# JonathanLehner/korali

Hardware: AMD Instinct MI355X
Metric: CMA-ES generations/sec + samples/sec, 128-dim Rosenbrock λ=4096, 1→8 GPUs (higher is better)
Workload: dtype f64; 1 GPU; C2: CMA-ES, 128-dim negative Rosenbrock, lambda=4096, mu=2048 Logarithmic, x0=0, sigma0=1, seed 1337; one experiment per GPU; population=4096, variables=128, covariance_update=exact, parallelism=replicas1

## Files before the change

### include/korali_amd.h

```cpp
#ifndef KORALI_AMD_H
#define KORALI_AMD_H

#include <stddef.h>
#include <stdint.h>

#ifdef __cplusplus
extern "C" {
#endif

#define KG_ABI_VERSION 8

const char *kg_last_error(void);
int kg_abi_version(void);
int kg_device_count(int *count);

typedef struct kg_cmaes_s *kg_cmaes_t;

enum kg_mu_type { KG_MU_LOGARITHMIC = 0, KG_MU_LINEAR = 1, KG_MU_EQUAL = 2, KG_MU_PROPORTIONAL = 3 };
enum kg_objective { KG_OBJ_NEGATIVE_ROSENBROCK = 0, KG_OBJ_NEGATIVE_ACKLEY = 1, KG_OBJ_NEGATIVE_SPHERE = 2 };
enum kg_cov_mode { KG_COV_EXACT = 0, KG_COV_MFMA = 1 };

typedef struct {
  size_t variable_count;
  size_t population_size;
// ... 11 lines not shown
  const double *initial_value;
  const double *initial_std;
  const double *min_std_update;
  uint64_t normal_seed;
  uint64_t uniform_seed;
  int cov_mode;
  int device;
  int store_bdz;
  int eigen_device_chase;
  int shard_rank;
  int shard_count;
  int use_gradients;
  double gradient_step_size;
  const double *granularity;
  size_t constraint_count;
  size_t viability_population_size;
  size_t viability_mu_value;
  double max_covariance_matrix_corrections;
  double target_success_rate;
  double covariance_matrix_adaption_strength;
  double global_success_learning_rate;
} kg_cmaes_cfg;

int kg_cmaes_create(const kg_cmaes_cfg *cfg, kg_cmaes_t *out);

typedef int (*kg_constraint_fn)(const double *X, size_t rows, size_t N, const size_t *ids, double *out, void *ctx);
int kg_cmaes_set_constraints(kg_cmaes_t h, kg_constraint_fn fn, void *ctx);
int kg_cmaes_prepare_constrained(kg_cmaes_t h, size_t generation);
int kg_cmaes_population_size(kg_cmaes_t h, size_t *lambda, size_t *mu);
int kg_cmaes_destroy(kg_cmaes_t h);
int kg_cmaes_initialize(kg_cmaes_t h);
int kg_cmaes_sample(kg_cmaes_t h);
int kg_cmaes_eval_builtin(kg_cmaes_t h, int objective);
int kg_cmaes_get_candidates(kg_cmaes_t h, double *X, size_t ld);
int kg_cmaes_set_fitness(kg_cmaes_t h, const double *F);
int kg_cmaes_set_log_posterior(kg_cmaes_t h, const double *F);
int kg_cmaes_set_gradients(kg_cmaes_t h, const double *G);
int kg_cmaes_update(kg_cmaes_t h, size_t generation);
int kg_cmaes_generation(kg_cmaes_t h, size_t generation, int objective);
int kg_cmaes_begin_sample(kg_cmaes_t h);
#define KG_TERMINATION_FIELDS 9
int kg_cmaes_wait_termination_fields(kg_cmaes_t h, double *out);
int kg_cmaes_update_partial(kg_cmaes_t h, size_t generation);
int kg_cmaes_shard_row_count(kg_cmaes_t h, size_t *count);
int kg_cmaes_update_rows(kg_cmaes_t h, size_t generation);
int kg_cmaes_update_finalize(kg_cmaes_t h, size_t generation);
int kg_cmaes_synchronize(kg_cmaes_t h);
int kg_cmaes_field_size(kg_cmaes_t h, const char *name, size_t *n);
int kg_cmaes_get_field(kg_cmaes_t h, const char *name, double *out, size_t n);
int kg_cmaes_set_field(kg_cmaes_t h, const char *name, const double *in, size_t n);
int kg_cmaes_get_fields(kg_cmaes_t h, const char *const *names, size_t count, double *out);
int kg_cmaes_get_sorting_index(kg_cmaes_t h, uint64_t *out);
int kg_cmaes_get_rng(kg_cmaes_t h, int which, void *state5000);
int kg_cmaes_set_rng(kg_cmaes_t h, int which, const void *state5000);
int kg_cmaes_device_ptr(kg_cmaes_t h, const char *name, void **ptr);
int kg_cmaes_stream(kg_cmaes_t h, void **stream);
int kg_cmaes_profile(kg_cmaes_t h, int enable);
int kg_cmaes_profile_read(kg_cmaes_t h, const char *stage, double *ms_total, size_t *count);
int kg_cmaes_profile_mark(kg_cmaes_t h, const char *stage, int phase);

typedef struct kg_dea_s *kg_dea_t;

enum kg_dea_mutation_rule { KG_DEA_MUTATION_FIXED = 0, KG_DEA_MUTATION_SELF_ADAPTIVE = 1 };
enum kg_dea_parent_rule { KG_DEA_PARENT_RANDOM = 0, KG_DEA_PARENT_BEST = 1 };
enum kg_dea_accept_rule {
  KG_DEA_ACCEPT_BEST = 0,
// ... 193 lines not shown
```

### korali_amd/csrc/kg_cmaes.hip

```cpp
#include <cmath>
#include <cstdio>
#include <cstdlib>
#include <cstring>
#include <map>
#include <string>
#include <tuple>
#include <vector>

#include "../../include/korali_amd.h"
#include "kg_common.hpp"
#include "kg_chains.hpp"
#include "kg_eigen.hpp"
#include "kg_rng.hpp"
#include <chrono>

namespace kg {


struct CmaesScalars {
  double sigma, trace, effectiveMu, cumulativeCovariance, sigmaCumulationFactor, dampFactor, chiSquareNumber;
  double psNorm, bestEverValue, previousBestEverValue, previousBestValue, currentBestValue;
  double currentMinStd, currentMaxStd, maxDiagC, minDiagC, minEig, maxEig;
  double infeasibleSampleCount, bestValidSample, modelEvaluationCount, hsig, eigenFailures;
  double ccov1, ccovmu;
// ... 99 lines not shown
      C[i * N + i] = v * v;
    }
    double mn = D[0], mx = D[0];
    for (int i = 1; i < N; i++) {
      if (D[i] < mn) mn = D[i];
      if (D[i] > mx) mx = D[i];
    }
    sc->minEig = mn * mn;
    sc->maxEig = mx * mx;
    double maxd = C[0], mind = C[0];
    for (int i = 1; i < N; ++i)
      if (maxd < C[i * N + i]) maxd = C[i * N + i];
    for (int i = 1; i < N; ++i)
      if (mind > C[i * N + i]) mind = C[i * N + i];
    sc->maxDiagC = maxd;
    sc->minDiagC = mind;
    if (full) {
      sc->infeasibleSampleCount = 0;
      sc->psNorm = 0.0;
      sc->currentMinStd = INFINITY;
      sc->currentMaxStd = -INFINITY;
      sc->hsigPowGen = -1.0;
    }
  }
}

constexpr int TR_BK = 32, TR_XCD = 8;
template <int BM, int BN>
inline unsigned tr_grid(int rows, int N) {
  const int nbm = (rows + BM - 1) / BM, nbn = (N + BN - 1) / BN;
  return (unsigned)(((nbm + TR_XCD - 1) / TR_XCD) * TR_XCD * nbn);
}
template <int BM, int BN>
__global__ void __launch_bounds__(256) k_transform(int N, int rows, int diagonal, const double *__restrict__ Z,
                                                   const double *__restrict__ B, const double *__restrict__ D,
                                                   const double *__restrict__ mean, CmaesScalars *__restrict__ sc,
                                                   const double *__restrict__ lb, const double *__restrict__ ub,
                                                   double *__restrict__ X, double *__restrict__ BDZ,
                                                   int *__restrict__ infeas, int no_reserve, int mirrored) {
  constexpr int PR = BM / 8, PC = BN / 32, ZL = BM * TR_BK / 256, BL = BN * TR_BK / 256;
  __shared__ __attribute__((aligned(16))) double Za[TR_BK][BM + 2];
  __shared__ __attribute__((aligned(16))) double Bt[TR_BK][BN + 2];
  const int tid = threadIdx.x;
  const int nbn = (N + BN - 1) / BN;
  const int xcd = blockIdx.x % TR_XCD, j = blockIdx.x / TR_XCD;
  const int rt = (j / nbn) * TR_XCD + xcd, ct = j % nbn;
  const int i0 = rt * BM, d0 = ct * BN;
  if (i0 >= rows) return;
  const int tx = tid & 31, ty = tid >> 5;
  const double sigma = sc->sigma;
  double acc[PR][PC];
#pragma unroll
  for (int p = 0; p < PR; p++)
#pragma unroll
    for (int q = 0; q < PC; q++) acc[p][q] = 0.0;
  if (!diagonal) {
    double zr[ZL], br[BL];
    auto load = [&](int k0) {
#pragma unroll
      for (int r = 0; r < ZL; r++) {
        const int q = tid + 256 * r, c = q / TR_BK, e = k0 + q % TR_BK, i = i0 + c;
        double z = 0.0;
        if (i < rows && e < N) {
          z = Z[(size_t)(mirrored ? (i >> 1) : i) * N + e];
          if (mirrored && (i & 1)) z = -z;
          z = D[e] * z;
        }
        zr[r] = z;
      }
#pragma unroll
      for (int r = 0; r < BL; r++) {
        const int q = tid + 256 * r, dd = q / TR_BK, e = k0 + q % TR_BK, d = d0 + dd;
        br[r] = (d < N && e < N) ? B[(size_t)d * N + e] : 0.0;
      }
    };
    auto store = [&]() {
#pragma unroll
      for (int r = 0; r < ZL; r++) {
        const int q = tid + 256 * r;
        Za[q % TR_BK][q / TR_BK] = zr[r];
      }
// ... 32 lines not shown
          for (int u = 0; u < 8; u++) t[u] = b[(g + u) % PC] * a[(g + u) / PC];
#pragma unroll
          for (int u = 0; u < 8; u++) acc[(g + u) / PC][(g + u) % PC] += t[u];
        }
      };
      fetch(a0, b0, 0);
      if (kmax == TR_BK) {
#pragma unroll 1
        for (int kk = 0; kk < TR_BK - 2; kk += 2) {
          fetch(a1, b1, kk + 1);
          madd(a0, b0);
          fetch(a0, b0, kk + 2);
          madd(a1, b1);
        }
        fetch(a1, b1, TR_BK - 1);
        madd(a0, b0);
        madd(a1, b1);
      } else {
#pragma unroll 1
        for (int kk = 0; kk < kmax; kk++) {
          fetch(a0, b0, kk);
          madd(a0, b0);
        }
      }
      __syncthreads();
      if (more) {
        store();
        __syncthreads();
      }
    }
  }
#pragma unroll
  for (int p = 0; p < PR; p++) {
    const int i = i0 + ty * PR + p;
    if (i >= rows) continue;
    int bad = 0;
#pragma unroll
    for (int q = 0; q < PC; q++) {
      const int d = d0 + tx * PC + q;
      if (d >= N) continue;
      double zd = 0.0;
      if (diagonal) {
        zd = Z[(size_t)(mirrored ? (i >> 1) : i) * N + d];
        if (mirrored && (i & 1)) zd = -zd;
      }
      const double bdz = diagonal ? D[d] * zd : acc[p][q];
      const double x = mean[d] + sigma * bdz;
      X[(size_t)i * N + d] = x;
      if (BDZ) BDZ[(size_t)i * N + d] = bdz;
      if (!isfinite(x) || x < lb[d] || x > ub[d]) bad = 1;
    }
    if (bad) {
      if (no_reserve)
        atomicOr(&sc->errors, KG_ERR_DRAW_GUARD);
      else
        atomicOr(&infeas[i], 1);
    }
  }
}

constexpr int PS_T = 64;
__global__ void __launch_bounds__(256) k_prescale_t(int N, int rows, int ldz, const double *__restrict__ Z,
                                                    const double *__restrict__ D, int mirrored,
                                                    double *__restrict__ dzT) {
  __shared__ double t[PS_T][PS_T + 1];
  const int i0 = blockIdx.x * PS_T, k0 = blockIdx.y * PS_T, tid = threadIdx.x;
#pragma unroll 4
  for (int r = 0; r < PS_T * PS_T / 256; r++) {
    const int q = tid + 256 * r, ii = q / PS_T, kk = q % PS_T, i = i0 + ii, k = k0 + kk;
    double z = 0.0;
    if (i < rows && k < N) {
      z = Z[(size_t)(mirrored ? (i >> 1) : i) * N + k];
      if (mirrored && (i & 1)) z = -z;
      z = D[k] * z;
    }
    t[ii][kk] = z;
  }
  __syncthreads();
#pragma unroll 4
  for (int r = 0; r < PS_T * PS_T / 256; r++) {
    const int q = tid + 256 * r, kk = q / PS_T, ii = q % PS_T, k = k0 + kk;
    if (k < N) dzT[(size_t)k * ldz + i0 + ii] = t[ii][kk];
  }
}
inline int sc_ldz(size_t rows) { return (int)((rows + 127) / 128 * 128); }
template <int C, int RPL>
inline unsigned trs_grid(int rows, int N) {
  const int nrt = (rows + 64 * RPL - 1) / (64 * RPL), ncg = (N + 4 * C - 1) / (4 * C);
  return (unsigned)(((nrt + TR_XCD - 1) / TR_XCD) * TR_XCD * ncg);
}
inline int transform_width(int N) {
// ... 188 lines not shown
        const int d = d0 + dd;
        if (obj == KG_OBJ_NEGATIVE_ROSENBROCK) {
          if (d > 0) {
            const double tt = x - prev * prev;
            const double u = 1 - prev;
            r0 += 100 * (tt * tt) + u * u;
          }
          prev = x;
        } else if (obj == KG_OBJ_NEGATIVE_ACKLEY) {
          r0 += x * x;
          r1 += ctile[tid][dd];
        } else {
          r0 += x * x;
        }
      }
    }
    __syncthreads();
  }
  if (tid >= OB_C || i >= lam) return;
  double f;
  if (obj == KG_OBJ_NEGATIVE_ROSENBROCK)
    f = -r0;
  else if (obj == KG_OBJ_NEGATIVE_ACKLEY) {
    const double s1 = r0 / (double)N, s2 = r1 / (double)N;
    const double e1 = 20. * exp_cr(-0.2 * sqrt(s1));
    const double e2 = exp_cr(s2);
    f = e1 + e2 - 20. - 2.718281828459045;
  } else
    f = -0.5 * r0;
  F[i] = f;
  if (!isfinite(f)) atomicOr(&sc->errors, KG_ERR_NONFINITE_F);
}

constexpr int OB2_R = 64, OB2_NC = 32;
__host__ __device__ inline size_t ob2_lds_bytes(int N) {
  return ((size_t)OB2_R * (N + 1) + 2 * 2 * (size_t)OB2_R * (OB2_NC + 1)) * sizeof(double);
}
__global__ void __launch_bounds__(256) k_objective2(int N, int lam, int obj, const double *__restrict__ X,
                                                    double *__restrict__ F, CmaesScalars *sc, double addEvals) {
  extern __shared__ __attribute__((aligned(16))) double ob2[];
  if (blockIdx.x == 0 && threadIdx.x == 0) sc->modelEvaluationCount += addEvals;
  const int tid = threadIdx.x, lane = tid & 63, wid = __builtin_amdgcn_readfirstlane(tid >> 6);
  const int ld = N + 1, c0 = blockIdx.x * OB2_R;
  double *Xs = ob2;
  double *Ta = Xs + (size_t)OB2_R * ld;
  double *Tb = Ta + 2 * (size_t)OB2_R * (OB2_NC + 1);
  const int tot = OB2_R * N;
  for (int q0 = tid; q0 < tot; q0 += 32 * 256) {
    double v[32];
#pragma unroll
    for (int u = 0; u < 32; u++) {
      const int q = q0 + u * 256, r = q / N, d = q - r * N;
      v[u] = (q < tot && c0 + r < lam) ? X[(size_t)(c0 + r) * N + d] : 0.0;
    }
#pragma unroll
    for (int u = 0; u < 32; u++) {
      const int q = q0 + u * 256, r = q / N, d = q - r * N;
      if (q < tot) Xs[(size_t)r * ld + d] = v[u];
    }
  }
  __syncthreads();
  const int nch = (N + OB2_NC - 1) / OB2_NC;
  const double cc = 2. * 3.141592653589793;
  auto form = [&](int ch) {
    const int b = ch & 1, d0 = ch * OB2_NC, dn = min(OB2_NC, N - d0);
    double *ta = Ta + (size_t)b * OB2_R * (OB2_NC + 1) + (size_t)lane * (OB2_NC + 1);
    double *tb = Tb + (size_t)b * OB2_R * (OB2_NC + 1) + (size_t)lane * (OB2_NC + 1);
    const double *xr = Xs + (size_t)lane * ld;
    if (obj != KG_OBJ_NEGATIVE_ACKLEY) {
      constexpr int PU = (OB2_NC + 2) / 3;
      double xs[PU], xp[PU];
#pragma unroll
      for (int u = 0; u < PU; u++) {
        const int dd = wid - 1 + 3 * u, d = d0 + dd;
        xs[u] = dd < dn ? xr[d] : 0.0;
        xp[u] = (dd < dn && d > 0) ? xr[d - 1] : 0.0;
      }
#pragma unroll
      for (int u = 0; u < PU; u++) {
        const int dd = wid - 1 + 3 * u, d = d0 + dd;
        if (dd >= dn) break;
        const double x = xs[u];
        if (obj == KG_OBJ_NEGATIVE_ROSENBROCK) {
          if (d > 0) {
            const double prev = xp[u];
            const double tt = x - prev * prev;
            const double uu = 1 - prev;
            ta[dd] = 100 * (tt * tt) + uu * uu;
          }
        } else {
          ta[dd] = x * x;
        }
      }
      return;
    }
    for (int dd = wid - 1; dd < dn; dd += 3) {
      const int d = d0 + dd;
      const double x = xr[d];
      if (obj == KG_OBJ_NEGATIVE_ROSENBROCK) {
        if (d > 0) {
          const double prev = xr[d - 1];
          const double tt = x - prev * prev;
          const double u = 1 - prev;
          ta[dd] = 100 * (tt * tt) + u * u;
        }
      } else if (obj == KG_OBJ_NEGATIVE_ACKLEY) {
        ta[dd] = x * x;
        tb[dd] = cos_cr(cc * x);
      } else {
        ta[dd] = x * x;
      }
    }
  };
  if (wid > 0) form(0);
  __syncthreads();
  double r0 = 0.0, r1 = 0.0;
  for (int ch = 0; ch < nch; ch++) {
    if (wid == 0) {
      const int b = ch & 1, d0 = ch * OB2_NC, dn = min(OB2_NC, N - d0);
      const double *ta = Ta + (size_t)b * OB2_R * (OB2_NC + 1) + (size_t)lane * (OB2_NC + 1);
      const double *tb = Tb + (size_t)b * OB2_R * (OB2_NC + 1) + (size_t)lane * (OB2_NC + 1);
      if (obj == KG_OBJ_NEGATIVE_ROSENBROCK) {
        int dd = d0 == 0 ? 1 : 0;
        for (; dd + 8 <= dn; dd += 8) {
          double t[8];
#pragma unroll
          for (int u = 0; u < 8; u++) t[u] = ta[dd + u];
#pragma unroll
          for (int u = 0; u < 8; u++) r0 += t[u];
        }
        for (; dd < dn; dd++) r0 += ta[dd];
      } else if (obj == KG_OBJ_NEGATIVE_ACKLEY) {
        for (int dd = 0; dd < dn; dd++) {
          r0 += ta[dd];
          r1 += tb[dd];
        }
      } else {
        for (int dd = 0; dd < dn; dd++) r0 += ta[dd];
      }
    } else if (ch + 1 < nch) {
      form(ch + 1);
    }
    __syncthreads();
  }
  const int i = c0 + lane;
  if (wid != 0 || i >= lam) return;
  double f;
  if (obj == KG_OBJ_NEGATIVE_ROSENBROCK)
    f = -r0;
  else if (obj == KG_OBJ_NEGATIVE_ACKLEY) {
    const double s1 = r0 / (double)N, s2 = r1 / (double)N;
    const double e1 = 20. * exp_cr(-0.2 * sqrt(s1));
    const double e2 = exp_cr(s2);
    f = e1 + e2 - 20. - 2.718281828459045;
  } else
    f = -0.5 * r0;
  F[i] = f;
  if (!isfinite(f)) atomicOr(&sc->errors, KG_ERR_NONFINITE_F);
}

constexpr int SORT_CHUNK = 2048;
__device__ inline bool before(double ka, unsigned ia, double kb, unsigned ib) {
  return (ka > kb) || (ka == kb && ia < ib);
}

__global__ void __launch_bounds__(1024) k_sort_init(int lam, int P2, const double *__restrict__ F, double *key,
                                                    unsigned *val) {
  const int i = blockIdx.x * blockDim.x + threadIdx.x;
  if (i >= P2) return;
  key[i] = (i < lam) ? F[i] : -INFINITY;
  val[i] = (i < lam) ? (unsigned)i : 0xffffffffu;
}

__global__ void __launch_bounds__(1024) k_sort_local(int P2, int kfixed, double *key, unsigned *val) {
  __shared__ double sk[SORT_CHUNK];
  __shared__ unsigned sv[SORT_CHUNK];
  const int base = blockIdx.x * SORT_CHUNK;
  for (int q = threadIdx.x; q < SORT_CHUNK; q += blockDim.x) {
    sk[q] = key[base + q];
    sv[q] = val[base + q];
  }
  __syncthreads();
  const int kstart = kfixed ? kfixed : 2, kend = kfixed ? kfixed : SORT_CHUNK;
  for (int k = kstart; k <= kend; k <<= 1) {
    const int jstart = kfixed ? SORT_CHUNK / 2 : k / 2;
    for (int j = jstart; j > 0; j >>= 1) {
      for (int q = threadIdx.x; q < SORT_CHUNK; q += blockDim.x) {
        const int l = q ^ j;
        if (l > q) {
// ... 2037 lines not shown
  double *covPart = nullptr, *Y = nullptr;
  double *Yc = nullptr, *Tt = nullptr;
  double *dzT = nullptr;
  size_t dzTRows = 0;
  int trW = 0;
  EigenSolver eig;
  int *infeas = nullptr, *assign = nullptr;
  int *selEnd = nullptr;
  unsigned long long *blockEnd = nullptr, *usedBlocks = nullptr;
  bool stateDirty = true;
  size_t resamplingRounds = 0;
  bool mirrored = false;
  double *G = nullptr;
  bool hasDiscrete = false;
  double *gran = nullptr, *mask = nullptr, *maskSigma = nullptr, *ubuf = nullptr, *dzero = nullptr;
  unsigned long long *uused = nullptr;
  size_t ucap = 0;
  size_t blocks = 0;
  int kslices = 8;
  int shards = 1, shardRank = 0, r0 = 0, r1 = 0;
  bool replSample = false;
  int *kidx = nullptr, *shardCnt = nullptr;
  double *part = nullptr;
  int *shardPos = nullptr, *shardCounts = nullptr;
  double *rows = nullptr, *covPack = nullptr;
  size_t rowsCap = 0;
  int rowBlock = -1;
  unsigned long long *eigTrace = nullptr;
  TermSummary *summary = nullptr, *summaryDev = nullptr;
  unsigned long long updates = 0;
  bool sampleBegun = false;
  bool consumePending = false;
  bool fusedSel = true, earlyPub = true;
  unsigned *meanArrived = nullptr;
  unsigned meanTarget = 0;
  MtStream normal, uniform;
  bool profile = false;
  std::vector<std::tuple<std::string, hipEvent_t, hipEvent_t>> pending;
  std::map<std::string, hipEvent_t> openMarks;
  std::map<std::string, std::pair<double, size_t>> prof;
};

namespace {

struct Stage {
  kg_cmaes_s *h;
  std::string name;
  hipEvent_t a = nullptr, b = nullptr;
  hipStream_t s;
  Stage(kg_cmaes_s *h_, const char *n, hipStream_t on = nullptr) : h(h_), name(n), s(on ? on : h_->stream) {
    if (h->profile) {
      (void)hipEventCreate(&a);
      (void)hipEventCreate(&b);
      (void)hipEventRecord(a, s);
    }
  }
  ~Stage() {
    if (h->profile) {
      (void)hipEventRecord(b, s);
      h->pending.emplace_back(name, a, b);
    }
  }
};

int flush_consume(kg_cmaes_s *h) {
  if (!h->consumePending) return 0;
// ... 358 lines not shown
    const size_t pbytes = ((size_t)N * (PA_EC + 1) + N) * sizeof(double);
    if (pbytes > 64 * 1024)
      KG_HIP(allow_dynamic_lds((const void *)k_paths, (int)pbytes));
    KG_HIP(allow_dynamic_lds((const void *)k_mean2, (int)mean2_lds_bytes()));
    if (N <= 128)
      KG_HIP(allow_dynamic_lds((const void *)k_objective2, (int)ob2_lds_bytes(N)));
    if (N <= 128)
      KG_HIP(allow_dynamic_lds((const void *)k_paths2, (int)paths2_lds_bytes(N)));
  }
  if (rc) {
    delete h;
    return 1;
  }
  KG_HIP(stream_acquire(&h->stream));
  KG_HIP(stream_acquire(&h->stream2));
  KG_HIP(hipEventCreateWithFlags(&h->evY, hipEventDisableTiming));
  KG_HIP(hipEventCreateWithFlags(&h->evC, hipEventDisableTiming));
  {
    const char *ev = getenv("KORALI_AMD_EIGEN_CHASE");
    bool hostChase = !cfg->eigen_device_chase;
    if (ev && std::string(ev) == "device") hostChase = false;
    if (ev && std::string(ev) == "host") hostChase = true;
    if (h->eig.init(N, hostChase)) {
      delete h;
      return 1;
    }
  }
  clk.mark("eigen");
  {
    const char *e = getenv("KORALI_AMD_FUSED_SELECT");
    h->fusedSel = !(e && *e == '0');
    e = getenv("KORALI_AMD_EARLY_PUBLISH");
    h->earlyPub = !(e && *e == '0');
  }
  if (set_current(h, h->lamCfg, h->muCfg)) return 1;
  KG_HIP(hipMemcpy(h->lb, lb.data(), N * sizeof(double), hipMemcpyHostToDevice));
  KG_HIP(hipMemcpy(h->ub, ub.data(), N * sizeof(double), hipMemcpyHostToDevice));
  KG_HIP(hipMemcpy(h->iv, iv.data(), N * sizeof(double), hipMemcpyHostToDevice));
  KG_HIP(hipMemcpy(h->istd, istd.data(), N * sizeof(double), hipMemcpyHostToDevice));
  KG_HIP(hipMemcpy(h->minstd, minstd.data(), N * sizeof(double), hipMemcpyHostToDevice));
  KG_HIP(hipMemcpy(h->gran, gran.data(), N * sizeof(double), hipMemcpyHostToDevice));
  KG_HIP(hipMemset(h->mask, 0, N * sizeof(double)));
  KG_HIP(hipMemset(h->maskSigma, 0, N * sizeof(double)));
  const size_t words = h->normal.words_for_normals(rows * N);
  if (h->normal.init(3 * words + 4096) || h->uniform.init(std::max<size_t>(1 << 16, 2 * h->ucap + 4096))) {
    delete h;
    return 1;
  }
  clk.mark("rng_init");
  unsigned char st[5000];
  gsl_seed_state(cfg->normal_seed, st);
  if (h->normal.import_gsl(st, h->stream)) return 1;
  clk.mark("normal_seed");
  gsl_seed_state(cfg->uniform_seed, st);
  if (h->uniform.import_gsl(st, h->stream)) return 1;
  clk.mark("uniform_seed");
  *out = h;
  return 0;
}

int kg_cmaes_destroy(kg_cmaes_t h) {
  if (!h) return 0;
  (void)flush_consume(h);
  (void)hipStreamSynchronize(h->stream);
  if (h->stream2) (void)hipStreamSynchronize(h->stream2);
  h->eig.drain();
// ... 204 lines not shown
    }
    int se[2] = {0, 0};
    KG_HIP(hipMemcpyAsync(se, h->selEnd, sizeof(se), hipMemcpyDeviceToHost, h->stream));
    KG_HIP(hipStreamSynchronize(h->stream));
    if (se[0] >= L) break;
    if (se[0] == i0) {
      if (se[1]) {
        const size_t cap = 2 * h->ucap;
        KG_CHECK(cap + 4096 <= h->uniform.capacity_words() / 2,
                 "discrete mutations need more uniforms per sample than the device window holds");
        double *nb2 = nullptr;
        if (dalloc(&nb2, cap)) return 1;
        dev_release(h->ubuf, h->stream);
        h->ubuf = nb2;
        h->ucap = cap;
      } else {
        bool fin = false, stateFinite = false;
        if (draw_guard(h, &fin, &stateFinite)) return 1;
        KG_CHECK(stateFinite, "the sampling distribution (mean, sigma, axis lengths) is not finite: every draw is "
                              "infeasible and the reference would redraw forever");
      }
    }
    i0 = se[0];
  }
  if (!h->R) {
    const unsigned long long used = (unsigned long long)nb;
    KG_HIP(hipMemcpyAsync(h->usedBlocks, &used, sizeof(used), hipMemcpyHostToDevice, h->stream));
  }
  return 0;
}

static bool plain_update(kg_cmaes_t h);

int kg_cmaes_sample(kg_cmaes_t h) {
  const int N = h->N;
  if (flush_consume(h)) return 1;
  if (!h->sampleBegun && cmaes_draw_begin(h)) return 1;
  h->sampleBegun = false;
  if (cmaes_eigen(h)) return 1;
  {
    Stage st(h, "rng_polar");
    if (h->normal.join(h->stream)) return 1;
  }
  bool redraw = h->R > 0;
  if (!redraw) {
    bool finite = false;
    if (draw_guard(h, &finite)) return 1;
    if (!finite) {
      KG_CHECK(h->shards == 1 || h->replSample,
               "a population-sharded handle cannot redraw non-finite samples (overflow guard tripped)");
      if (ensure_redraw_buffers(h)) return 1;
      redraw = true;
    }
  }
  if (redraw) return cmaes_resample(h);
  {
    Stage st(h, "transform");
    const int t0 = h->replSample ? 0 : h->r0, t1 = h->replSample ? h->lam : h->r1;
    const size_t trows = (size_t)(t1 - t0);
    double *xo = h->X + (size_t)t0 * N;
    double *bo = h->BDZ ? h->BDZ + (size_t)t0 * N : nullptr;
    if (cmaes_transform(h, trows, xo, bo, 1, h->mirrored ? 1 : 0)) return 1;
  }
  h->consumePending = true;
  if (!plain_update(h)) return flush_consume(h);
  return 0;
}

int kg_cmaes_eval_builtin(kg_cmaes_t h, int objective) {
  KG_CHECK(objective >= 0 && objective <= 2, "unknown builtin objective");
  Stage st(h, "objective");
  const int rows = h->r1 - h->r0;
  if (h->N <= 128)
    hipLaunchKernelGGL(k_objective2, dim3((rows + OB2_R - 1) / OB2_R), dim3(256), ob2_lds_bytes(h->N), h->stream,
                       h->N, rows, objective, h->X + (size_t)h->r0 * h->N, h->F + h->r0, h->sc, (double)h->lam);
  else
    hipLaunchKernelGGL(k_objective, dim3((rows + OB_C - 1) / OB_C), dim3(256), 0, h->stream, h->N, rows, objective,
                       h->X + (size_t)h->r0 * h->N, h->F + h->r0, h->sc, (double)h->lam);
  KG_HIP(hipGetLastError());
  return 0;
}

int kg_cmaes_get_candidates(kg_cmaes_t h, double *X, size_t ld) {
  const size_t N = h->N;
  if (ld == 0) ld = N;
  KG_HIP(hipMemcpy2DAsync(X, ld * sizeof(double), h->X, N * sizeof(double), N * sizeof(double), h->lam,
                          hipMemcpyDeviceToHost, h->stream));
  KG_HIP(hipStreamSynchronize(h->stream));
  return 0;
}

static int cmaes_upload_fitness(kg_cmaes_t h, const double *F, bool allow_neg_inf) {
  for (int i = 0; i < h->lam; i++)
    KG_CHECK(std::isfinite(F[i]) || (allow_neg_inf && F[i] == -INFINITY),
             "Non finite value of function evaluation detected: " + std::to_string(F[i]));
  KG_HIP(hipMemcpyAsync(h->F, F, h->lam * sizeof(double), hipMemcpyHostToDevice, h->stream));
  hipLaunchKernelGGL(k_add_evals, dim3(1), dim3(1), 0, h->stream, h->sc, (double)h->lam);
  KG_HIP(hipStreamSynchronize(h->stream));
  return 0;
// ... 506 lines not shown
  const int N = h->N;
  if (h->covPack) {
    Stage st(h, "covariance");
    hipLaunchKernelGGL(k_shard_cov_unpack, dim3(N), dim3(256), 0, h->stream, N, (const double *)h->covPack, h->C);
    KG_HIP(hipGetLastError());
    if (early_publish(h)) return 1;
    if (flush_consume(h)) return 1;
    return cmaes_sigma(h, generation);
  }
  {
    Stage st(h, "mean_paths");
    hipLaunchKernelGGL(k_shard_finalize, dim3((N + 255) / 256), dim3(256), 0, h->stream, N, h->part, h->mean,
                       h->prevMean, h->meanUpdate, h->currBestVars, h->bestEverVars, h->sc);
    if (h->G)
      hipLaunchKernelGGL(k_mean_gradient, dim3((N + 63) / 64), dim3(64), 0, h->stream, N, h->mu,
                         h->cfg.gradient_step_size, h->G, h->idx, h->w, h->mean, h->prevMean, h->meanUpdate, h->sc);
    KG_HIP(hipGetLastError());
    if (cmaes_paths(h, generation)) return 1;
  }
  {
    Stage st(h, "covariance");
    const int nt = (N + 15) / 16, ntiles = nt * (nt + 1) / 2;
    hipLaunchKernelGGL(k_adaptC_combine, dim3(ntiles), dim3(256), 0, h->stream, N, 1, ntiles,
                       h->cfg.diagonal_covariance, h->part + 2 * (size_t)N, h->pc, h->C, h->sc, 1);
    KG_HIP(hipGetLastError());
  }
  if (flush_consume(h)) return 1;
  return cmaes_sigma(h, generation);
}

int kg_cmaes_generation(kg_cmaes_t h, size_t generation, int objective) {
  KG_CHECK(h->shards == 1, "a population-sharded generation needs the caller's collectives between its stages");
  if (generation == 1 && kg_cmaes_initialize(h)) return 1;
  if (kg_cmaes_sample(h)) return 1;
  if (kg_cmaes_eval_builtin(h, objective)) return 1;
  return kg_cmaes_update(h, generation);
}

int kg_cmaes_wait_termination_fields(kg_cmaes_t h, double *out) {
  const unsigned long long want = h->updates;
  KG_CHECK(want > 0, "kg_cmaes_wait_termination_fields before any kg_cmaes_update");
  const auto t0 = std::chrono::steady_clock::now();
  while (__atomic_load_n(&h->summary->seq, __ATOMIC_ACQUIRE) < want) {
    __builtin_ia32_pause();
    if (std::chrono::steady_clock::now() - t0 > std::chrono::seconds(60)) {
      KG_HIP(hipStreamSynchronize(h->stream));
      if (check_errors(h)) return 1;
      KG_CHECK(false, "termination summary never arrived");
    }
  }
  if (h->summary->errors) {
    KG_HIP(hipStreamSynchronize(h->stream));
    return check_errors(h);
  }
  for (int i = 0; i < KG_TERMINATION_FIELDS; i++) out[i] = h->summary->f[i];
  return 0;
}

int kg_cmaes_synchronize(kg_cmaes_t h) {
  if (flush_consume(h)) return 1;
  KG_HIP(hipStreamSynchronize(h->stream));
  if (h->eigTrace) {
    unsigned long long t[32];
    KG_HIP(hipMemcpy(t, h->eigTrace, sizeof(t), hipMemcpyDeviceToHost));
    int steps = 0, rots = 0;
    h->eig.last_counts(steps, rots);
    fprintf(stderr,
            "[korali_amd tridiag trace, cumulative s_memtime ticks] nrm2 %llu dsymv %llu xv %llu dsyr2 %llu; last QR: "
// ... 266 lines not shown
```

### korali_amd/engine/engine.cpp

```cpp
#include <algorithm>
#include <atomic>
#include <cctype>
#include <chrono>
#include <cmath>
#include <condition_variable>
#include <cstdarg>
#include <cstdio>
#include <cstring>
#include <exception>
#include <fstream>
#include <functional>
#include <memory>
#include <mutex>
#include <random>
#include <sstream>
#include <thread>
#include <sys/stat.h>
#include <unistd.h>

#include "../../include/korali_amd.h"
#include "distributed.hpp"
#include "korali.hpp"

namespace korali {
// ... 967 lines not shown
  void evaluateConstraints(const double *x, size_t N_, double *out) {
    Sample s;
    s["Module"] = "Problem";
    s["Operation"] = "Evaluate Constraints";
    s["Sample Id"] = (unsigned long long)0;
    s["Current Generation"] = (unsigned long long)curGen;
    s["Parameters"] = std::vector<double>(x, x + N_);
    for (size_t c = 0; c < constraintFns.size(); c++) {
      getFunction(constraintFns[c])(s);
      if (!s.contains("F(x)")) fail("The constraint function %zu did not assign 'F(x)'.", c);
      const double v = s["F(x)"].getDouble();
      if (!std::isfinite(v)) fail("Non finite value of constraint evaluation %lu detected: %f\n", (unsigned long)c, v);
      out[c] = v;
    }
  }
  std::exception_ptr pendingError;

  void runGeneration(size_t gen) override {
    curGen = gen;
    if (gen == 1) check(kg_cmaes_initialize(h));
    if (!constraintFns.empty()) {
      if (kg_cmaes_prepare_constrained(h, gen) != 0) {
        if (pendingError) {
          std::exception_ptr e = pendingError;
          pendingError = nullptr;
          std::rethrow_exception(e);
        }
        check(1);
      }
      size_t cur = 0;
      check(kg_cmaes_population_size(h, &cur, nullptr));
      lam = cur;
      r1 = lam;
    } else {
      check(kg_cmaes_sample(h));
    }
    if (objective >= 0) {
      check(kg_cmaes_eval_builtin(h, objective));
    } else if (replicated) {
      splitEvaluate(gen);
    } else if (dist) {
      hostEvaluate(gen, r0, r1);
    } else {
      std::vector<double> X(lam * N), F(lam), G(useGradients ? lam * N : 0);
      check(kg_cmaes_get_candidates(h, X.data(), N));
      Function *f = bayesian ? nullptr : &getFunction(fn);
      conduit->evaluateBatch(lam, [&](size_t i) { evaluateSample(gen, i, X, F, G, f); });
      check(bayesian ? kg_cmaes_set_log_posterior(h, F.data()) : kg_cmaes_set_fitness(h, F.data()));
      if (useGradients) check(kg_cmaes_set_gradients(h, G.data()));
    }
    if (dist && !replicated) {
      auto mark = [&](const char *stage, int phase) {
        if (exchangeProfile) check(kg_cmaes_profile_mark(h, stage, phase));
      };
      mark("exchange_fitness", 0);
      dist->allGather(buffer("Value Vector"), r1 - r0);
      if (useGradients) dist->allGather(buffer("Gradients"), (r1 - r0) * N);
      mark("exchange_fitness", 1);
      check(kg_cmaes_update_partial(h, gen));
      size_t n = 0;
      if (exactShards) {
        check(kg_cmaes_shard_row_count(h, &n));
        mark("exchange_rows", 0);
        if (n) dist->allGather(buffer("Shard Rows"), n);
        mark("exchange_rows", 1);
        check(kg_cmaes_update_rows(h, gen));
        check(kg_cmaes_field_size(h, "Shard Covariance", &n));
        mark("exchange_covariance", 0);
        dist->allReduceMaxI64(buffer("Shard Covariance"), n);
        mark("exchange_covariance", 1);
      } else {
// ... 1492 lines not shown
```

### korali_amd/native.py

```python
import ctypes as C
import os

import numpy as np

_PKG = os.path.dirname(os.path.abspath(__file__))
LIB_PATH = os.path.join(_PKG, "libkorali_amd.so")
if os.environ.get("KORALI_AMD_LIB_VARIANT"):
    LIB_PATH = os.path.join(_PKG, f"libkorali_amd_{os.environ['KORALI_AMD_LIB_VARIANT']}.so")
_LIB = None

MU_TYPES = {"logarithmic": 0, "linear": 1, "equal": 2, "proportional": 3}
OBJECTIVES = {"negative rosenbrock": 0, "negative ackley": 1, "negative sphere": 2,
              "rosenbrock": 0, "ackley": 1, "sphere": 2}
COV_MODES = {"exact": 0, "mfma": 1}


class KoraliDeviceError(RuntimeError):
    pass


class _CmaesCfg(C.Structure):
    _fields_ = [
        ("variable_count", C.c_size_t), ("population_size", C.c_size_t), ("mu_value", C.c_size_t),
        ("mu_type", C.c_int), ("initial_sigma_cumulation_factor", C.c_double),
# ... 35 lines not shown


class _TmcmcHierarchical(C.Structure):
    _fields_ = [
        ("mode", C.c_int), ("prior_count", C.c_size_t), ("kind", C.POINTER(C.c_int)),
        ("param_index", C.POINTER(C.c_int)), ("param_const", C.POINTER(C.c_double)),
        ("group_count", C.c_size_t), ("group_size", C.POINTER(C.c_size_t)), ("row_width", C.c_size_t),
        ("rows", C.POINTER(C.c_double)), ("log_prior", C.POINTER(C.c_double)),
    ]


HIER_MODES = {"psi": 0, "thetanew": 1}
PRIOR_KINDS = {"uniform": 0, "normal": 1, "exponential": 2, "laplace": 3, "cauchy": 4, "lognormal": 5}


class _DeaCfg(C.Structure):
    _fields_ = [
        ("variable_count", C.c_size_t), ("population_size", C.c_size_t),
        ("lower_bound", C.POINTER(C.c_double)), ("upper_bound", C.POINTER(C.c_double)),
        ("crossover_rate", C.c_double), ("mutation_rate", C.c_double), ("mutation_rule", C.c_int),
        ("parent_rule", C.c_int), ("accept_rule", C.c_int), ("fix_infeasible", C.c_int),
        ("normal_seed", C.c_uint64), ("uniform_seed", C.c_uint64), ("window_words", C.c_size_t),
        ("max_windows", C.c_size_t), ("device", C.c_int),
    ]


DEA_MUTATION_RULES = {"fixed": 0, "self adaptive": 1}
DEA_PARENT_RULES = {"random": 0, "best": 1}
DEA_ACCEPT_RULES = {"best": 0, "greedy": 1, "iterative": 2, "improved": 3}

EXPORTED = [
    "kg_last_error", "kg_abi_version", "kg_device_count",
    "kg_cmaes_create", "kg_cmaes_destroy", "kg_cmaes_initialize", "kg_cmaes_sample", "kg_cmaes_eval_builtin",
    "kg_cmaes_get_candidates", "kg_cmaes_set_fitness", "kg_cmaes_set_log_posterior", "kg_cmaes_update", "kg_cmaes_generation",
    "kg_cmaes_begin_sample", "kg_cmaes_wait_termination_fields", "kg_cmaes_set_gradients", "kg_cmaes_update_partial", "kg_cmaes_update_finalize",
    "kg_cmaes_shard_row_count", "kg_cmaes_update_rows",
    "kg_cmaes_synchronize", "kg_cmaes_field_size", "kg_cmaes_get_field", "kg_cmaes_set_field",
    "kg_cmaes_get_fields", "kg_cmaes_get_sorting_index", "kg_cmaes_get_rng", "kg_cmaes_set_rng", "kg_cmaes_device_ptr",
    "kg_cmaes_stream", "kg_cmaes_profile", "kg_cmaes_profile_read", "kg_cmaes_profile_mark",
    "kg_cmaes_set_constraints", "kg_cmaes_prepare_constrained", "kg_cmaes_population_size",
    "kg_dea_create", "kg_dea_destroy", "kg_dea_initialize", "kg_dea_prepare", "kg_dea_eval_builtin",
    "kg_dea_get_candidates", "kg_dea_set_fitness", "kg_dea_update", "kg_dea_generation", "kg_dea_synchronize",
    "kg_dea_field_size", "kg_dea_get_field", "kg_dea_set_field", "kg_dea_get_rng", "kg_dea_set_rng",
    "kg_dea_windows", "kg_dea_profile", "kg_dea_profile_read",
    "kg_tmcmc_create", "kg_tmcmc_destroy", "kg_tmcmc_generation", "kg_tmcmc_synchronize", "kg_tmcmc_field_size",
    "kg_tmcmc_get_field", "kg_tmcmc_set_field", "kg_tmcmc_get_rng", "kg_tmcmc_set_rng", "kg_tmcmc_prepare",
    "kg_tmcmc_evaluate", "kg_tmcmc_process", "kg_tmcmc_advance", "kg_tmcmc_get_pending",
    "kg_tmcmc_process_partial", "kg_tmcmc_process_finalize", "kg_tmcmc_device_ptr", "kg_tmcmc_stream", "kg_tmcmc_evaluate_prior", "kg_tmcmc_get_candidates", "kg_tmcmc_set_evaluations",
    "kg_tmcmc_set_gradients", "kg_tmcmc_set_hierarchical", "kg_tmcmc_hierarchical_loglik",
    "kg_tmcmc_profile", "kg_tmcmc_profile_read", "kg_debug_mt_jump", "kg_debug_multinomial", "kg_debug_cartpole",
    "kg_debug_cartpole_at",
    "kg_debug_host_tridiag", "kg_debug_host_chase",
    "kg_vracer_create", "kg_vracer_destroy", "kg_vracer_hyperparameter_count", "kg_vracer_field_size",
    "kg_vracer_get_field", "kg_vracer_set_field", "kg_vracer_get_scalar", "kg_vracer_set_scalar",
    "kg_vracer_run_policy", "kg_vracer_set_action_noise", "kg_vracer_environment_step", "kg_vracer_train_policy",
    "kg_vracer_train_policy_minibatch", "kg_vracer_training_step", "kg_vracer_test_episodes", "kg_vracer_rescale_states", "kg_vracer_synchronize", "kg_vracer_stream",
    "kg_vracer_profile", "kg_vracer_profile_read", "kg_vracer_save_state", "kg_vracer_load_state",
    "kg_vracer_train_pending", "kg_vracer_host_launch", "kg_vracer_host_act", "kg_vracer_host_feed",
]


def lib():
    global _LIB
    if _LIB is None:
        if not os.path.exists(LIB_PATH):
            raise KoraliDeviceError(f"{LIB_PATH} not built; run `python -m korali_amd._build` (hipcc, gfx950)")
        L = C.CDLL(LIB_PATH)
        vp, sz, dp, cp, ip = C.c_void_p, C.c_size_t, C.POINTER(C.c_double), C.c_char_p, C.c_int
        L.kg_last_error.restype = cp
        L.kg_abi_version.restype = ip
        L.kg_device_count.argtypes = [C.POINTER(C.c_int)]
        L.kg_cmaes_create.argtypes = [C.POINTER(_CmaesCfg), C.POINTER(vp)]
        for f in ("kg_cmaes_destroy", "kg_cmaes_initialize", "kg_cmaes_sample", "kg_cmaes_synchronize",
                  "kg_cmaes_begin_sample"):
            getattr(L, f).argtypes = [vp]
        L.kg_cmaes_eval_builtin.argtypes = [vp, ip]
        L.kg_cmaes_get_candidates.argtypes = [vp, dp, sz]
        L.kg_cmaes_set_fitness.argtypes = [vp, dp]
        L.kg_cmaes_set_log_posterior.argtypes = [vp, dp]
        L.kg_cmaes_set_gradients.argtypes = [vp, dp]
        L.kg_cmaes_update.argtypes = [vp, sz]
        L.kg_cmaes_update_partial.argtypes = [vp, sz]
        L.kg_cmaes_update_finalize.argtypes = [vp, sz]
        L.kg_cmaes_shard_row_count.argtypes = [vp, C.POINTER(sz)]
        L.kg_cmaes_update_rows.argtypes = [vp, sz]
        L.kg_debug_mt_jump.argtypes = [vp, C.c_uint64, vp]
        L.kg_debug_multinomial.argtypes = [C.c_uint64, C.c_size_t, C.c_uint, vp, C.c_size_t, vp, vp]
        L.kg_debug_cartpole.argtypes = [ip, vp, vp, sz, sz, vp, vp]
        L.kg_debug_cartpole_at.argtypes = [ip, vp, vp, vp, sz, sz, vp, vp, vp]
        L.kg_debug_host_tridiag.argtypes = [sz, vp, vp, vp, vp, vp]
        L.kg_debug_host_chase.argtypes = [sz, vp, vp, C.c_int, sz, vp, vp, vp, sz, vp, vp]
        L.kg_cmaes_generation.argtypes = [vp, sz, ip]
        L.kg_cmaes_field_size.argtypes = [vp, cp, C.POINTER(sz)]
        L.kg_cmaes_get_field.argtypes = [vp, cp, dp, sz]
        L.kg_cmaes_set_field.argtypes = [vp, cp, dp, sz]
        L.kg_cmaes_get_sorting_index.argtypes = [vp, C.POINTER(C.c_uint64)]
        L.kg_cmaes_get_fields.argtypes = [vp, C.POINTER(cp), sz, dp]
        L.kg_cmaes_wait_termination_fields.argtypes = [vp, dp]
        L.kg_cmaes_set_constraints.argtypes = [vp, CONSTRAINT_FN, vp]
        L.kg_cmaes_prepare_constrained.argtypes = [vp, sz]
        L.kg_cmaes_population_size.argtypes = [vp, C.POINTER(sz), C.POINTER(sz)]
        L.kg_cmaes_get_rng.argtypes = [vp, ip, vp]
        L.kg_cmaes_set_rng.argtypes = [vp, ip, vp]
        L.kg_cmaes_device_ptr.argtypes = [vp, cp, C.POINTER(vp)]
        L.kg_cmaes_stream.argtypes = [vp, C.POINTER(vp)]
        L.kg_cmaes_profile.argtypes = [vp, ip]
        L.kg_cmaes_profile_read.argtypes = [vp, cp, dp, C.POINTER(sz)]
        L.kg_cmaes_profile_mark.argtypes = [vp, cp, ip]
        L.kg_dea_create.argtypes = [C.POINTER(_DeaCfg), C.POINTER(vp)]
# ... 126 lines not shown
            self._cfn = CONSTRAINT_FN(cb)
            check(L.kg_cmaes_set_constraints(self.h, self._cfn, None))

    @property
    def lam(self):
        n = C.c_size_t()
        check(self._L.kg_cmaes_population_size(self.h, C.byref(n), None))
        return n.value

    def prepare_constrained(self, generation):
        check(self._L.kg_cmaes_prepare_constrained(self.h, int(generation)))

    def close(self):
        if getattr(self, "h", None):
            self._L.kg_cmaes_destroy(self.h)
            self.h = None

    def __del__(self):
        try:
            self.close()
        except Exception:
            pass

    def initialize(self):
        check(self._L.kg_cmaes_initialize(self.h))

    def sample(self):
        check(self._L.kg_cmaes_sample(self.h))

    def evaluate(self, objective):
        check(self._L.kg_cmaes_eval_builtin(self.h, OBJECTIVES[objective.lower()] if isinstance(objective, str)
                                            else int(objective)))

    def update(self, generation):
        check(self._L.kg_cmaes_update(self.h, int(generation)))

    def update_partial(self, generation):
        check(self._L.kg_cmaes_update_partial(self.h, int(generation)))

    def update_finalize(self, generation):
        check(self._L.kg_cmaes_update_finalize(self.h, int(generation)))

    def shard_row_count(self):
        n = C.c_size_t(0)
        check(self._L.kg_cmaes_shard_row_count(self.h, C.byref(n)))
        return int(n.value)

    def update_rows(self, generation):
        check(self._L.kg_cmaes_update_rows(self.h, int(generation)))

    def begin_sample(self):
        check(self._L.kg_cmaes_begin_sample(self.h))

    def generation(self, generation, objective):
        obj = OBJECTIVES[objective.lower()] if isinstance(objective, str) else int(objective)
        check(self._L.kg_cmaes_generation(self.h, int(generation), obj))

    def synchronize(self):
        check(self._L.kg_cmaes_synchronize(self.h))

    def candidates(self):
        X = np.empty((self.lam, self.N))
        check(self._L.kg_cmaes_get_candidates(self.h, _dptr(X), self.N))
        return X

    def _fitness_arg(self, F):
# ... 359 lines not shown
```

Measured before the change: 1984 generations/s.

## Fuse candidate transform with builtin objective evaluation in one kernel

Moves the sampling transform body into a device helper and adds a kernel that computes X = mean + sigma·B·D·Z for a 16-row tile spanning all N≤128 columns, then evaluates the Rosenbrock/Ackley/sphere objective from the tile held in shared memory and writes F directly. This drops a separate objective kernel launch and its re-read of X from global memory. It only applies in the single-shard, unconstrained, unbounded, non-diagonal case, and can be disabled with an environment variable. The narrow BM=16 tile may lower GEMM efficiency compared with the generic transform tiling.

Measured after the change: 2022 generations/s (median of 6 runs). +1.9%, better.

```diff
diff --git a/include/korali_amd.h b/include/korali_amd.h
--- a/include/korali_amd.h
+++ b/include/korali_amd.h
@@ -67,6 +67,7 @@
 int kg_cmaes_initialize(kg_cmaes_t h);
 int kg_cmaes_sample(kg_cmaes_t h);
 int kg_cmaes_eval_builtin(kg_cmaes_t h, int objective);
+int kg_cmaes_sample_eval(kg_cmaes_t h, int objective);
 int kg_cmaes_get_candidates(kg_cmaes_t h, double *X, size_t ld);
 int kg_cmaes_set_fitness(kg_cmaes_t h, const double *F);
 int kg_cmaes_set_log_posterior(kg_cmaes_t h, const double *F);
diff --git a/korali_amd/csrc/kg_cmaes.hip b/korali_amd/csrc/kg_cmaes.hip
--- a/korali_amd/csrc/kg_cmaes.hip
+++ b/korali_amd/csrc/kg_cmaes.hip
@@ -155,21 +155,21 @@
   return (unsigned)(((nbm + TR_XCD - 1) / TR_XCD) * TR_XCD * nbn);
 }
 template <int BM, int BN>
-__global__ void __launch_bounds__(256) k_transform(int N, int rows, int diagonal, const double *__restrict__ Z,
-                                                   const double *__restrict__ B, const double *__restrict__ D,
-                                                   const double *__restrict__ mean, CmaesScalars *__restrict__ sc,
-                                                   const double *__restrict__ lb, const double *__restrict__ ub,
-                                                   double *__restrict__ X, double *__restrict__ BDZ,
-                                                   int *__restrict__ infeas, int no_reserve, int mirrored) {
+__device__ __forceinline__ bool tr_tile(int N, int rows, int diagonal, const double *__restrict__ Z,
+                                        const double *__restrict__ B, const double *__restrict__ D,
+                                        const double *__restrict__ mean, CmaesScalars *__restrict__ sc,
+                                        const double *__restrict__ lb, const double *__restrict__ ub,
+                                        double *__restrict__ X, double *__restrict__ BDZ, int *__restrict__ infeas,
+                                        int no_reserve, int mirrored, double (&Za)[TR_BK][BM + 2],
+                                        double (&Bt)[TR_BK][BN + 2], int &i0, double (&xo)[BM / 8][BN / 32]) {
   constexpr int PR = BM / 8, PC = BN / 32, ZL = BM * TR_BK / 256, BL = BN * TR_BK / 256;
-  __shared__ __attribute__((aligned(16))) double Za[TR_BK][BM + 2];
-  __shared__ __attribute__((aligned(16))) double Bt[TR_BK][BN + 2];
   const int tid = threadIdx.x;
   const int nbn = (N + BN - 1) / BN;
   const int xcd = blockIdx.x % TR_XCD, j = blockIdx.x / TR_XCD;
   const int rt = (j / nbn) * TR_XCD + xcd, ct = j % nbn;
-  const int i0 = rt * BM, d0 = ct * BN;
-  if (i0 >= rows) return;
+  const int d0 = ct * BN;
+  i0 = rt * BM;
+  if (i0 >= rows) return false;
   const int tx = tid & 31, ty = tid >> 5;
   const double sigma = sc->sigma;
   double acc[PR][PC];
@@ -268,6 +268,8 @@
   }
 #pragma unroll
   for (int p = 0; p < PR; p++) {
+#pragma unroll
+    for (int q = 0; q < PC; q++) xo[p][q] = 0.0;
     const int i = i0 + ty * PR + p;
     if (i >= rows) continue;
     int bad = 0;
@@ -283,6 +285,7 @@
       const double bdz = diagonal ? D[d] * zd : acc[p][q];
       const double x = mean[d] + sigma * bdz;
       X[(size_t)i * N + d] = x;
+      xo[p][q] = x;
       if (BDZ) BDZ[(size_t)i * N + d] = bdz;
       if (!isfinite(x) || x < lb[d] || x > ub[d]) bad = 1;
     }
@@ -293,6 +296,21 @@
         atomicOr(&infeas[i], 1);
     }
   }
+  return true;
+}
+template <int BM, int BN>
+__global__ void __launch_bounds__(256) k_transform(int N, int rows, int diagonal, const double *__restrict__ Z,
+                                                   const double *__restrict__ B, const double *__restrict__ D,
+                                                   const double *__restrict__ mean, CmaesScalars *__restrict__ sc,
+                                                   const double *__restrict__ lb, const double *__restrict__ ub,
+                                                   double *__restrict__ X, double *__restrict__ BDZ,
+                                                   int *__restrict__ infeas, int no_reserve, int mirrored) {
+  __shared__ __attribute__((aligned(16))) double Za[TR_BK][BM + 2];
+  __shared__ __attribute__((aligned(16))) double Bt[TR_BK][BN + 2];
+  int i0;
+  double xo[BM / 8][BN / 32];
+  (void)tr_tile<BM, BN>(N, rows, diagonal, Z, B, D, mean, sc, lb, ub, X, BDZ, infeas, no_reserve, mirrored, Za, Bt, i0,
+                        xo);
 }
 
 constexpr int PS_T = 64;
@@ -547,6 +565,27 @@
   if (!isfinite(f)) atomicOr(&sc->errors, KG_ERR_NONFINITE_F);
 }
 
+__device__ __forceinline__ double obj_rosenbrock_term(double x, double prev) {
+  const double tt = x - prev * prev;
+  const double uu = 1 - prev;
+  return 100 * (tt * tt) + uu * uu;
+}
+__device__ __forceinline__ double obj_square_term(double x) { return x * x; }
+__device__ __forceinline__ double obj_ackley_cos_term(double x) {
+  const double cc = 2. * 3.141592653589793;
+  return cos_cr(cc * x);
+}
+__device__ __forceinline__ double obj_value(int obj, int N, double r0, double r1) {
+  if (obj == KG_OBJ_NEGATIVE_ROSENBROCK) return -r0;
+  if (obj == KG_OBJ_NEGATIVE_ACKLEY) {
+    const double s1 = r0 / (double)N, s2 = r1 / (double)N;
+    const double e1 = 20. * exp_cr(-0.2 * sqrt(s1));
+    const double e2 = exp_cr(s2);
+    return e1 + e2 - 20. - 2.718281828459045;
+  }
+  return -0.5 * r0;
+}
+
 constexpr int OB2_R = 64, OB2_NC = 32;
 __host__ __device__ inline size_t ob2_lds_bytes(int N) {
   return ((size_t)OB2_R * (N + 1) + 2 * 2 * (size_t)OB2_R * (OB2_NC + 1)) * sizeof(double);
@@ -576,7 +615,6 @@
   }
   __syncthreads();
   const int nch = (N + OB2_NC - 1) / OB2_NC;
-  const double cc = 2. * 3.141592653589793;
   auto form = [&](int ch) {
     const int b = ch & 1, d0 = ch * OB2_NC, dn = min(OB2_NC, N - d0);
     double *ta = Ta + (size_t)b * OB2_R * (OB2_NC + 1) + (size_t)lane * (OB2_NC + 1);
@@ -597,34 +635,17 @@
         if (dd >= dn) break;
         const double x = xs[u];
         if (obj == KG_OBJ_NEGATIVE_ROSENBROCK) {
-          if (d > 0) {
-            const double prev = xp[u];
-            const double tt = x - prev * prev;
-            const double uu = 1 - prev;
-            ta[dd] = 100 * (tt * tt) + uu * uu;
-          }
+          if (d > 0) ta[dd] = obj_rosenbrock_term(x, xp[u]);
         } else {
-          ta[dd] = x * x;
+          ta[dd] = obj_square_term(x);
         }
       }
       return;
     }
     for (int dd = wid - 1; dd < dn; dd += 3) {
-      const int d = d0 + dd;
-      const double x = xr[d];
-      if (obj == KG_OBJ_NEGATIVE_ROSENBROCK) {
-        if (d > 0) {
-          const double prev = xr[d - 1];
-          const double tt = x - prev * prev;
-          const double u = 1 - prev;
-          ta[dd] = 100 * (tt * tt) + u * u;
-        }
-      } else if (obj == KG_OBJ_NEGATIVE_ACKLEY) {
-        ta[dd] = x * x;
-        tb[dd] = cos_cr(cc * x);
-      } else {
-        ta[dd] = x * x;
-      }
+      const double x = xr[d0 + dd];
+      ta[dd] = obj_square_term(x);
+      tb[dd] = obj_ackley_cos_term(x);
     }
   };
   if (wid > 0) form(0);
@@ -660,16 +681,79 @@
   }
   const int i = c0 + lane;
   if (wid != 0 || i >= lam) return;
-  double f;
-  if (obj == KG_OBJ_NEGATIVE_ROSENBROCK)
-    f = -r0;
-  else if (obj == KG_OBJ_NEGATIVE_ACKLEY) {
-    const double s1 = r0 / (double)N, s2 = r1 / (double)N;
-    const double e1 = 20. * exp_cr(-0.2 * sqrt(s1));
-    const double e2 = exp_cr(s2);
-    f = e1 + e2 - 20. - 2.718281828459045;
-  } else
-    f = -0.5 * r0;
+  const double f = obj_value(obj, N, r0, r1);
+  F[i] = f;
+  if (!isfinite(f)) atomicOr(&sc->errors, KG_ERR_NONFINITE_F);
+}
+
+constexpr int TO_BM = 16, TO_BN = 128;
+__global__ void __launch_bounds__(256) k_transform_obj(int N, int rows, const double *__restrict__ Z,
+                                                       const double *__restrict__ B, const double *__restrict__ D,
+                                                       const double *__restrict__ mean, CmaesScalars *__restrict__ sc,
+                                                       const double *__restrict__ lb, const double *__restrict__ ub,
+                                                       double *__restrict__ X, double *__restrict__ BDZ,
+                                                       int *__restrict__ infeas, int mirrored, int obj,
+                                                       double *__restrict__ F, double addEvals) {
+  constexpr int PR = TO_BM / 8, PC = TO_BN / 32;
+  __shared__ __attribute__((aligned(16))) double Za[TR_BK][TO_BM + 2];
+  __shared__ __attribute__((aligned(16))) double Bt[TR_BK][TO_BN + 2];
+  static_assert(2 * TO_BM * (TO_BN + 1) <= TR_BK * (TO_BN + 2), "x tile + one term tile fit in Bt");
+  int i0;
+  double x[PR][PC];
+  if (!tr_tile<TO_BM, TO_BN>(N, rows, 0, Z, B, D, mean, sc, lb, ub, X, BDZ, infeas, 1, mirrored, Za, Bt, i0, x)) return;
+  const int tid = threadIdx.x, tx = tid & 31, ty = tid >> 5, ld = N + 1;
+  if (blockIdx.x == 0 && tid == 0) sc->modelEvaluationCount += addEvals;
+  double *Xs = &Bt[0][0];
+  double *Ta = Xs + TO_BM * ld;
+  if (obj == KG_OBJ_NEGATIVE_ROSENBROCK) {
+#pragma unroll
+    for (int p = 0; p < PR; p++)
+#pragma unroll
+      for (int q = 0; q < PC; q++) {
+        const int d = tx * PC + q;
+        if (d < N) Xs[(ty * PR + p) * ld + d] = x[p][q];
+      }
+    __syncthreads();
+  }
+#pragma unroll
+  for (int p = 0; p < PR; p++)
+#pragma unroll
+    for (int q = 0; q < PC; q++) {
+      const int r = ty * PR + p, d = tx * PC + q;
+      if (d >= N) continue;
+      if (obj == KG_OBJ_NEGATIVE_ROSENBROCK) {
+        if (d > 0) Ta[r * ld + d] = obj_rosenbrock_term(x[p][q], Xs[r * ld + d - 1]);
+      } else {
+        Ta[r * ld + d] = obj_square_term(x[p][q]);
+        if (obj == KG_OBJ_NEGATIVE_ACKLEY) Xs[r * ld + d] = obj_ackley_cos_term(x[p][q]);
+      }
+    }
+  __syncthreads();
+  const int i = i0 + tid;
+  if (tid >= TO_BM || i >= rows) return;
+  const double *ta = Ta + tid * ld, *tb = Xs + tid * ld;
+  double r0 = 0.0, r1 = 0.0;
+  int d = obj == KG_OBJ_NEGATIVE_ROSENBROCK ? 1 : 0;
+  if (obj == KG_OBJ_NEGATIVE_ACKLEY) {
+    for (; d + 8 <= N; d += 8) {
+      double t[8], c[8];
+#pragma unroll
+      for (int u = 0; u < 8; u++) t[u] = ta[d + u], c[u] = tb[d + u];
+#pragma unroll
+      for (int u = 0; u < 8; u++) r0 += t[u], r1 += c[u];
+    }
+    for (; d < N; d++) r0 += ta[d], r1 += tb[d];
+  } else {
+    for (; d + 8 <= N; d += 8) {
+      double t[8];
+#pragma unroll
+      for (int u = 0; u < 8; u++) t[u] = ta[d + u];
+#pragma unroll
+      for (int u = 0; u < 8; u++) r0 += t[u];
+    }
+    for (; d < N; d++) r0 += ta[d];
+  }
+  const double f = obj_value(obj, N, r0, r1);
   F[i] = f;
   if (!isfinite(f)) atomicOr(&sc->errors, KG_ERR_NONFINITE_F);
 }
@@ -2773,6 +2857,7 @@
   bool sampleBegun = false;
   bool consumePending = false;
   bool fusedSel = true, earlyPub = true;
+  bool fusedDraw = true;
   unsigned *meanArrived = nullptr;
   unsigned meanTarget = 0;
   MtStream normal, uniform;
@@ -3197,6 +3282,8 @@
     h->fusedSel = !(e && *e == '0');
     e = getenv("KORALI_AMD_EARLY_PUBLISH");
     h->earlyPub = !(e && *e == '0');
+    e = getenv("KORALI_AMD_FUSED_DRAW");
+    h->fusedDraw = !(e && *e == '0');
   }
   if (set_current(h, h->lamCfg, h->muCfg)) return 1;
   KG_HIP(hipMemcpy(h->lb, lb.data(), N * sizeof(double), hipMemcpyHostToDevice));
@@ -3467,11 +3554,26 @@
 
 static bool plain_update(kg_cmaes_t h);
 
-int kg_cmaes_sample(kg_cmaes_t h) {
+static bool fused_draw(kg_cmaes_t h, int objective) {
+  return h->fusedDraw && objective >= 0 && objective <= 2 && h->N <= TO_BN && !h->cfg.diagonal_covariance &&
+         h->shards == 1 && h->R == 0 && !h->finiteBounds && !h->hasDiscrete && h->nc == 0 && h->trW == 0;
+}
+static int cmaes_transform_obj(kg_cmaes_t h, int objective) {
+  Stage st(h, "transform");
+  hipLaunchKernelGGL(k_transform_obj, dim3(tr_grid<TO_BM, TO_BN>(h->lam, h->N)), dim3(256), 0, h->stream, h->N, h->lam,
+                     h->Z, h->B, h->D, h->mean, h->sc, h->lb, h->ub, h->X, h->BDZ, h->infeas, h->mirrored ? 1 : 0,
+                     objective, h->F, (double)h->lam);
+  KG_HIP(hipGetLastError());
+  return 0;
+}
+
+static int cmaes_sample(kg_cmaes_t h, int objective, bool *evaluated) {
   const int N = h->N;
+  *evaluated = false;
   if (flush_consume(h)) return 1;
   if (!h->sampleBegun && cmaes_draw_begin(h)) return 1;
   h->sampleBegun = false;
+  const bool fused = fused_draw(h, objective);
   if (cmaes_eigen(h)) return 1;
   {
     Stage st(h, "rng_polar");
@@ -3489,7 +3591,10 @@
     }
   }
   if (redraw) return cmaes_resample(h);
-  {
+  if (fused) {
+    if (cmaes_transform_obj(h, objective)) return 1;
+    *evaluated = true;
+  } else {
     Stage st(h, "transform");
     const int t0 = h->replSample ? 0 : h->r0, t1 = h->replSample ? h->lam : h->r1;
     const size_t trows = (size_t)(t1 - t0);
@@ -3500,6 +3605,18 @@
   h->consumePending = true;
   if (!plain_update(h)) return flush_consume(h);
   return 0;
+}
+
+int kg_cmaes_sample(kg_cmaes_t h) {
+  bool evaluated = false;
+  return cmaes_sample(h, -1, &evaluated);
+}
+
+int kg_cmaes_sample_eval(kg_cmaes_t h, int objective) {
+  KG_CHECK(objective >= 0 && objective <= 2, "unknown builtin objective");
+  bool evaluated = false;
+  if (cmaes_sample(h, objective, &evaluated)) return 1;
+  return evaluated ? 0 : kg_cmaes_eval_builtin(h, objective);
 }
 
 int kg_cmaes_eval_builtin(kg_cmaes_t h, int objective) {
@@ -4072,8 +4189,7 @@
 int kg_cmaes_generation(kg_cmaes_t h, size_t generation, int objective) {
   KG_CHECK(h->shards == 1, "a population-sharded generation needs the caller's collectives between its stages");
   if (generation == 1 && kg_cmaes_initialize(h)) return 1;
-  if (kg_cmaes_sample(h)) return 1;
-  if (kg_cmaes_eval_builtin(h, objective)) return 1;
+  if (kg_cmaes_sample_eval(h, objective)) return 1;
   return kg_cmaes_update(h, generation);
 }
 
diff --git a/korali_amd/engine/engine.cpp b/korali_amd/engine/engine.cpp
--- a/korali_amd/engine/engine.cpp
+++ b/korali_amd/engine/engine.cpp
@@ -1023,11 +1023,13 @@
       check(kg_cmaes_population_size(h, &cur, nullptr));
       lam = cur;
       r1 = lam;
+    } else if (objective >= 0 && !dist) {
+      check(kg_cmaes_sample_eval(h, objective));
     } else {
       check(kg_cmaes_sample(h));
     }
     if (objective >= 0) {
-      check(kg_cmaes_eval_builtin(h, objective));
+      if (!constraintFns.empty() || dist) check(kg_cmaes_eval_builtin(h, objective));
     } else if (replicated) {
       splitEvaluate(gen);
     } else if (dist) {
diff --git a/korali_amd/native.py b/korali_amd/native.py
--- a/korali_amd/native.py
+++ b/korali_amd/native.py
@@ -91,6 +91,7 @@
 EXPORTED = [
     "kg_last_error", "kg_abi_version", "kg_device_count",
     "kg_cmaes_create", "kg_cmaes_destroy", "kg_cmaes_initialize", "kg_cmaes_sample", "kg_cmaes_eval_builtin",
+    "kg_cmaes_sample_eval",
     "kg_cmaes_get_candidates", "kg_cmaes_set_fitness", "kg_cmaes_set_log_posterior", "kg_cmaes_update", "kg_cmaes_generation",
     "kg_cmaes_begin_sample", "kg_cmaes_wait_termination_fields", "kg_cmaes_set_gradients", "kg_cmaes_update_partial", "kg_cmaes_update_finalize",
     "kg_cmaes_shard_row_count", "kg_cmaes_update_rows",
@@ -134,6 +135,7 @@
                   "kg_cmaes_begin_sample"):
             getattr(L, f).argtypes = [vp]
         L.kg_cmaes_eval_builtin.argtypes = [vp, ip]
+        L.kg_cmaes_sample_eval.argtypes = [vp, ip]
         L.kg_cmaes_get_candidates.argtypes = [vp, dp, sz]
         L.kg_cmaes_set_fitness.argtypes = [vp, dp]
         L.kg_cmaes_set_log_posterior.argtypes = [vp, dp]
@@ -326,6 +328,10 @@
         check(self._L.kg_cmaes_eval_builtin(self.h, OBJECTIVES[objective.lower()] if isinstance(objective, str)
                                             else int(objective)))
 
+    def sample_eval(self, objective):
+        check(self._L.kg_cmaes_sample_eval(self.h, OBJECTIVES[objective.lower()] if isinstance(objective, str)
+                                           else int(objective)))
+
     def update(self, generation):
         check(self._L.kg_cmaes_update(self.h, int(generation)))
 
```
